# Gabisanth/MaximumAreaCoverageOptimization.jl

Hardware: AMD Instinct MI355X
Metric: MADS objective evals/sec (N UAVs × M fire cells), 1/2/4/8 MI355X (higher is better)
Workload: dtype f64

## Files before the change

### maximumareacoverageoptimization.jl_amd/csrc/k_final.h

```cpp
#pragma once

#include <hip/hip_runtime.h>
#include <stdint.h>

#include "predicate.h"
#include "k_common.h"
#include "k_prep.h"

#pragma clang fp contract(off)

namespace mac {

#ifndef MAC_FIN_C
#define MAC_FIN_C 16
#endif
constexpr int kFinC = MAC_FIN_C;
#ifndef MAC_FIN_MAXBLK
#define MAC_FIN_MAXBLK 256
#endif
constexpr int kFinMaxBlk = MAC_FIN_MAXBLK;
constexpr int kFinThreads = 1024;

struct FinBest {
    double* best;
    uint64_t* mirror;
    uint64_t seq;
    int64_t idx_base;
    unsigned long long* blk;
    unsigned* arrive;
    MadsState* st;
    const double* x;
    double* x_next;
    const int* rp;
    const int* cp;
    uint64_t state;
    int n, ell_max;
    uint64_t done_seq;
    int* hint;
    int* hint_host;
    int nhint;
    int np;
    const unsigned long long* feas;
};

__host__ __device__ __forceinline__ uint64_t mirror_check(uint64_t o, uint64_t i, uint64_t q, uint64_t f = 0)
{
    uint64_t z = o ^ (i * 0x9E3779B97F4A7C15ull) ^ (q * 0xC2B2AE3D27D4EB4Full) ^ (f * 0xD6E8FEB86659FD93ull) ^
                 0x5851F42D4C957F2Dull;
    z = (z ^ (z >> 30)) * 0xBF58476D1CE4E5B9ull;
    z = (z ^ (z >> 27)) * 0x94D049BB133111EBull;
    return z ^ (z >> 31);
}

template <bool kXY = false, bool kMesh = false>
__device__ __forceinline__ void mads_step(const FinBest& fb, double bo, int64_t gidx, int ell, double f)
{
    const int lane = threadIdx.x & (kWave - 1);
    const int n = fb.n;
    const int np = kXY ? fb.np : n;
    const double* __restrict__ x = fb.x;
    double* __restrict__ xn = fb.x_next;
    const bool better = gidx >= 0 && bo < f;
    constexpr int kB = 8;
    const int64_t b = (int64_t)1 << ell;
    const bool plus = gidx < np;
    const int c = better ? fb.cp[plus ? (int)gidx : (int)gidx - np] : 0;
    [[maybe_unused]] const double* gran = nullptr;
    if constexpr (kMesh) gran = fb.st->gran;
    for (int v0 = lane; v0 < n; v0 += kB * kWave) {
        double xv[kB];
        [[maybe_unused]] double gv[kB];
        int rv[kB];
#pragma unroll
        for (int j = 0; j < kB; ++j) {
            const int v = v0 + j * kWave;
            xv[j] = v < n ? x[v] : 0.0;
            rv[j] = better && v < np ? fb.rp[v] : 0;
            if constexpr (kMesh) gv[j] = better && v < np ? gran[v] : 1.0;
        }
#pragma unroll
        for (int j = 0; j < kB; ++j) {
            const int v = v0 + j * kWave;
            if (v >= n) break;
            if (better) {
                double d = ltmads_entry(fb.state, np, b, rv[j], c);
                if constexpr (kMesh) d = gv[j] * d;
                const double moved = plus ? xv[j] + d : xv[j] - d;
                xn[v] = v < np ? moved : xv[j];
            } else {
                xn[v] = xv[j];
            }
        }
    }
    if (lane == 0) {
        const int e = better ? (ell + 1 < fb.ell_max ? ell + 1 : fb.ell_max) : ell - 1;
        fb.st->f = better ? bo : f;
        fb.st->ell = e;
        fb.st->it += 1;
        if (better) fb.st->succ += 1;
    }
}

__device__ __forceinline__ void argmin_take(double& v1, int& i1, double v2, int i2)
{
    if ((i2 >= 0) && (i1 < 0 || v2 < v1 || (v2 == v1 && i2 < i1))) {
        v1 = v2;
        i1 = i2;
    }
}

template <int C = kFinC, bool kXY = false, bool kMesh = false>
__device__ __forceinline__ bool finalize_argmin(const FinBest& fb, double o, int k, bool have)
{
    static_assert(C >= 1 && C <= kWave && (C & (C - 1)) == 0, "C: a power of two up to a wave");
    const int lane = threadIdx.x & (kWave - 1);
    double bv = __builtin_inf();
    int bi = -1;
    if (have && lane < C && o < bv) {
        bv = o;
        bi = k;
    }
#pragma unroll
    for (int off = C / 2; off >= 1; off >>= 1)
        argmin_take(bv, bi, __shfl_xor(bv, off, kWave), __shfl_xor(bi, off, kWave));
    unsigned old = 0;
    if (lane == 0) {
        __hip_atomic_store(fb.blk + 2 * blockIdx.x, __builtin_bit_cast(unsigned long long, bv),
                           __ATOMIC_RELAXED, __HIP_MEMORY_SCOPE_AGENT);
        __hip_atomic_store(fb.blk + 2 * blockIdx.x + 1, (unsigned long long)(long long)bi,
                           __ATOMIC_RELAXED, __HIP_MEMORY_SCOPE_AGENT);
        asm volatile("s_waitcnt vmcnt(0)" ::: "memory");
        old = __hip_atomic_fetch_add(fb.arrive, 1u, __ATOMIC_RELAXED, __HIP_MEMORY_SCOPE_AGENT);
    }
    old = __shfl(old, 0, kWave);
    if (old != gridDim.x - 1) return false;
    const int ell = fb.st ? fb.st->ell : 0;
    const double fcur = fb.st ? fb.st->f : 0.0;
    const int rej = fb.st ? fb.st->skip : 0;
    bv = __builtin_inf();
    bi = -1;
    constexpr int kPer = kFinMaxBlk / kWave;
    unsigned long long v[kPer], ix[kPer];
#pragma unroll
    for (int r = 0; r < kPer; ++r) {
        const unsigned q = lane + r * kWave;
        v[r] = q < gridDim.x ? __hip_atomic_load(fb.blk + 2 * q, __ATOMIC_RELAXED, __HIP_MEMORY_SCOPE_AGENT)
                             : __builtin_bit_cast(unsigned long long, __builtin_inf());
        ix[r] = q < gridDim.x ? __hip_atomic_load(fb.blk + 2 * q + 1, __ATOMIC_RELAXED, __HIP_MEMORY_SCOPE_AGENT)
                              : ~0ull;
    }
    const uint64_t fe = fb.feas ? __hip_atomic_load(fb.feas, __ATOMIC_RELAXED, __HIP_MEMORY_SCOPE_AGENT) : 0ull;
    const bool hl = fb.hint && lane < fb.nhint;
    const int hv = hl ? __hip_atomic_load(fb.hint + lane, __ATOMIC_RELAXED, __HIP_MEMORY_SCOPE_AGENT) : 0;
#pragma unroll
    for (int r = 0; r < kPer; ++r)
        if ((long long)ix[r] >= 0) argmin_take(bv, bi, __builtin_bit_cast(double, v[r]), (int)(long long)ix[r]);
    for (unsigned q = lane + kFinMaxBlk; q < gridDim.x; q += kWave) {
        const unsigned long long vv = __hip_atomic_load(fb.blk + 2 * q, __ATOMIC_RELAXED,
                                                        __HIP_MEMORY_SCOPE_AGENT);
        const unsigned long long xx = __hip_atomic_load(fb.blk + 2 * q + 1, __ATOMIC_RELAXED,
                                                        __HIP_MEMORY_SCOPE_AGENT);
        argmin_take(bv, bi, __builtin_bit_cast(double, vv), (int)(long long)xx);
    }
#pragma unroll
    for (int off = 32; off >= 1; off >>= 1)
        argmin_take(bv, bi, __shfl_xor(bv, off, kWave), __shfl_xor(bi, off, kWave));
    const bool none = bi < 0 || rej;
    const double bo = none ? __builtin_inf() : bv;
    const int64_t gidx = none ? (int64_t)-1 : fb.idx_base + bi;
    if (fb.st && ell < 0) {
        if (lane == 0) __hip_atomic_store(fb.arrive, 0u, __ATOMIC_RELAXED, __HIP_MEMORY_SCOPE_AGENT);
        return true;
    }
    if (fb.st) {
        mads_step<kXY, kMesh>(fb, bo, gidx, ell, fcur);
        if (rej && lane == 0) fb.st->skipped += 1;
    }
    if (lane == 0) {
        unsigned long long* const bw = reinterpret_cast<unsigned long long*>(fb.best);
        __hip_atomic_store(bw, __builtin_bit_cast(unsigned long long, bo), __ATOMIC_RELAXED,
                           __HIP_MEMORY_SCOPE_AGENT);
        __hip_atomic_store(bw + 1, (unsigned long long)gidx, __ATOMIC_RELAXED, __HIP_MEMORY_SCOPE_AGENT);
        __hip_atomic_store(fb.arrive, 0u, __ATOMIC_RELAXED, __HIP_MEMORY_SCOPE_AGENT);
        if (fb.mirror) {
            asm volatile("s_waitcnt vmcnt(0)" ::: "memory");
            const uint64_t o = __builtin_bit_cast(uint64_t, bo);
            const uint64_t ix = (uint64_t)gidx;
            fb.mirror[0] = o;
            fb.mirror[1] = ix;
            fb.mirror[2] = fb.seq;
            if (fb.feas) fb.mirror[4] = fe;
            fb.mirror[3] = mirror_check(o, ix, fb.seq, fe);
            if (fb.st && !(gidx >= 0 && bo < fcur) && ell == 0) fb.mirror[2] = fb.done_seq;
        }
    }
    if (hl) {
        if (fb.hint_host) ((volatile int*)fb.hint_host)[lane] = hv;
        __hip_atomic_store(fb.hint + lane, 0, __ATOMIC_RELAXED, __HIP_MEMORY_SCOPE_AGENT);
    }
    return true;
}

template <bool kXY = false, bool kMesh = false>
__global__ __launch_bounds__(kFinThreads) void finalize_kernel(
    const double* __restrict__ partial, const int* __restrict__ mode, int n_poll, int n_other,
    int K, int N, const int* __restrict__ map, const double* __restrict__ spart,
    const int* __restrict__ ncount, int counts, double w0,
    const double* __restrict__ vp, double* __restrict__ area_out, double* __restrict__ obj_out,
    FinBest fb, uint64_t* ts)
{
    ts_begin(ts);
    double o = __builtin_inf();
    __shared__ double red[kFinThreads / kFinC][kFinC];
    const int t = threadIdx.x, c = t % kFinC, sg = t / kFinC;
    constexpr int SG = kFinThreads / kFinC;
    const int per = (int)(gridDim.x / 8);
    const int cb = per > 0 && gridDim.x % 8 == 0 ? (int)(blockIdx.x % 8) * per + (int)(blockIdx.x / 8)
                                                 : (int)blockIdx.x;
    const int k0 = cb * kFinC;
    const int k = k0 + c;
    const int mv = mode ? *mode : 0;
    const bool cnt_path = counts && spart && map;
    const double vpk = (vp && (sg == 0 || cnt_path) && k < K) ? vp[k] : 0.0;
    if (cnt_path) {
        constexpr int B = 8;
        int pos0[B];
        bool sh0[B];
#pragma unroll
        for (int b = 0; b < B; ++b) {
            const int gb = sg + b * SG;
            const bool in = k < K && gb < n_poll;
            pos0[b] = in ? map[(int64_t)gb * K + k] : -1;
            sh0[b] = in && ncount[gb] > 0;
        }
        const bool skip = vp && !area_out && !(vpk < __builtin_inf());
        if (mv == kModePoll) {
            const unsigned* const crow = reinterpret_cast<const unsigned*>(partial);
            const unsigned* const srow = reinterpret_cast<const unsigned*>(spart);
            __shared__ uint64_t ired[kFinThreads / kFinC][kFinC];
            const int G = n_poll;
            uint64_t a = 0;
            if (k < K && !skip) {
                for (int g = sg; g < G; g += B * SG) {
                    unsigned v[B], sv[B];
                    int pos[B];
                    bool sh[B];
#pragma unroll
                    for (int b = 0; b < B; ++b) {
                        const int gb = g + b * SG;
                        if (g == sg) {
                            pos[b] = pos0[b];
                            sh[b] = sh0[b];
                        } else {
                            pos[b] = gb < G ? map[(int64_t)gb * K + k] : -1;
                            sh[b] = gb < G && ncount[gb] > 0;
                        }
                    }
#pragma unroll
                    for (int b = 0; b < B; ++b) {
                        const int64_t rb = (int64_t)(g + b * SG) * K;
                        v[b] = pos[b] >= 0 ? crow[rb + pos[b]] : 0u;
                        sv[b] = sh[b] ? srow[rb + k] : 0u;
                    }
#pragma unroll
                    for (int b = 0; b < B; ++b) a += (uint64_t)v[b] + sv[b];
                }
            }
            ired[sg][c] = a;
// ... 100 lines not shown
```

### maximumareacoverageoptimization.jl_amd/csrc/k_fiw.h

```cpp
#pragma once

#include <hip/hip_runtime.h>
#include <stdint.h>

#include <type_traits>

#include "predicate.h"
#include "fiw_box.h"
#include "k_common.h"
#include "k_prep.h"
#include "k_index.h"
#include "k_lane.h"
#include "k_poll.h"
#include "k_poll_shared.h"
#include "k_final.h"

#pragma clang fp contract(off)

namespace mac {

constexpr int kFwThreads = 256;
constexpr int kFwWaves = kFwThreads / kWave;
constexpr int kFwPer = 12;
constexpr int kFwMaxK = kFwThreads * kFwPer;
// ... 100 lines not shown
__device__ uint64_t g_diag_f2[8 * 4096];
#define MAC_F2_STAMP(q)                                                                      \
    if (threadIdx.x == 0 && blockIdx.x < 4096) {                                             \
        asm volatile("s_waitcnt vmcnt(0) lgkmcnt(0)" ::: "memory");                          \
        g_diag_f2[8 * blockIdx.x + (q)] = __builtin_amdgcn_s_memrealtime();                  \
    }
#define MAC_F2_NOW() __builtin_amdgcn_s_memrealtime()
#define MAC_F2_PUT(q, v) if (threadIdx.x == 0 && blockIdx.x < 4096) g_diag_f2[8 * blockIdx.x + (q)] = (v)
#else
#define MAC_FW_STAMP(q)
#define MAC_F2_STAMP(q)
#define MAC_F2_NOW() 0
#define MAC_F2_PUT(q, v)
#endif

template <bool C> struct FwAcc { typedef double T; };
template <> struct FwAcc<true> { typedef unsigned T; };

template <bool kCounts, bool kMat, bool kMesh = false>
__global__ __launch_bounds__(kFwThreads) __attribute__((amdgpu_waves_per_eu(2))) void fiw_kernel(
    uint64_t* ts, FwArgs a)
{
    typedef typename FwAcc<kCounts>::T Acc;
    ts_begin(ts);
    CandSrc src = a.src;
    const int N = a.N, K = a.K;
    const Grid g = a.g;
    const int per_xcd = (N + 7) / 8;
    const int i = (int)(blockIdx.x % 8) * per_xcd + (int)(blockIdx.x / 8);
    if (i >= N || !src.resolve_as<kMat>()) {
        ts_end(ts);
        return;
    }
    MAC_FW_STAMP(0);
    __shared__ __attribute__((aligned(16))) uint32_t xbuf[kFwMaxK + 1];
    __shared__ __attribute__((aligned(16))) double tabbuf[kFwMaxK + 1];
    __shared__ __attribute__((aligned(8))) uint16_t zbuf[kFwMaxK + 1];
    constexpr int kSl4 = kFwKPB * 16, kSlx = kFwKPB * 4, kS32 = (kFwCH + 4) * 16, kSix = kFwCH * 4,
                  kSw = kFwCH * 8;
    constexpr int kWB = kSl4 + kSlx + kS32 + kSix + kSw;
    __shared__ __attribute__((aligned(16))) unsigned char wbuf[kWB];
    static_assert(sizeof(uint64_t) * (kFwMaxK + 1) <= kWB, "coverage words fit the walk buffer");
    static_assert(sizeof(int) * (kFwDirect + 1) <= sizeof(double) * (kFwMaxK + 1), "direct table fits");
    constexpr int kFwClr = 4 * kFwThreads;
    __shared__ double2 shp[kFwShE];
    __shared__ double shw[kFwShE];
    __shared__ int shidx[kFwCH];
    __shared__ int rs[kPollRB], rpre[kPollRB + 1];
    __shared__ int nb_id[kFwNbr];
    __shared__ int4 nb_box[kFwNbr];
    __shared__ double nb_b[kFwNbr][3];
    __shared__ double dred[kFwWaves][4];
    __shared__ double sbase[7];
    __shared__ uint8_t scov[kFwKPB];
    __shared__ unsigned ninner;
    __shared__ int ucnt, ncnt, lslot;
    __shared__ int wkeep[kFwR][kFwWaves];
    __shared__ int wshr[kFwR][kFwWaves];
    __shared__ int wsum[kFwWaves];
    uint32_t* const kx = xbuf;
    uint32_t* const poskey = xbuf;
    int* const table = reinterpret_cast<int*>(tabbuf);
    unsigned* const pcnt = reinterpret_cast<unsigned*>(tabbuf);
    double* const pcred = tabbuf;
    uint16_t* const owner_of = reinterpret_cast<uint16_t*>(wbuf);
    uint16_t* const cinfo = zbuf;
    float4* const sl4 = reinterpret_cast<float4*>(wbuf);
    float* const slx = reinterpret_cast<float*>(wbuf + kSl4);
    float4* const s32 = reinterpret_cast<float4*>(wbuf + kSl4 + kSlx);
    int* const six = reinterpret_cast<int*>(wbuf + kSl4 + kSlx + kS32);
    double* const sw = reinterpret_cast<double*>(wbuf + kSl4 + kSlx + kS32 + kSix);
    uint64_t* const Wd = reinterpret_cast<uint64_t*>(wbuf);

    const int tid = threadIdx.x, lane = tid & (kWave - 1), wid = tid / kWave;
    constexpr int P = kFwPer + 1;
    auto kof = [&](int j) { return j < kFwPer ? tid * kFwPer + j : (tid == 0 ? kFwMaxK : K); };

    int4 RG = make_int4(0, -1, 0, -1);
    bool ident;
    int rf0 = 0, rf1 = 0;
    double2 ppr[kFwR];
    double pwr[kFwR];
    int pjg[kFwR];
    {
        const uint32_t* krow = src.keysP + (int64_t)i * src.ldk;
        uint32_t pq[P];
        bool dj[P];
#pragma unroll
        for (int c = 0; c < kFwPer / 4; ++c) {
            const int b0 = tid * kFwPer + 4 * c;
            const uint4 q4 = b0 < src.ldk ? *reinterpret_cast<const uint4*>(krow + b0) : make_uint4(0, 0, 0, 0);
            const uint32_t d4 = a.dead && b0 < src.ldk ? *reinterpret_cast<const uint32_t*>(a.dead + b0) : 0u;
            pq[4 * c] = q4.x;
            pq[4 * c + 1] = q4.y;
            pq[4 * c + 2] = q4.z;
            pq[4 * c + 3] = q4.w;
#pragma unroll
            for (int e = 0; e < 4; ++e) dj[4 * c + e] = ((d4 >> (8 * e)) & 0xFFu) != 0 && b0 + e < K;
        }
        pq[kFwPer] = tid == 0 && K > kFwMaxK ? krow[kFwMaxK] : 0u;
        dj[kFwPer] = tid == 0 && K > kFwMaxK && a.dead && a.dead[kFwMaxK] != 0;
        const double bx = src_val<kMat, kMesh>(src, 0, i, N), by = src_val<kMat, kMesh>(src, 0, N + i, N),
                     br = src_val<kMat, kMesh>(src, 0, 2 * N + i, N);
        double dmx = -__builtin_inf(), dmy = -__builtin_inf(), dmr = -__builtin_inf(), dml = -__builtin_inf();
        for (int q = tid; q < a.npd; q += kFwThreads) {
            const double4 d4 = a.pd[q];
            dmx = fmax(dmx, d4.x);
            dmy = fmax(dmy, d4.y);
            dmr = fmax(dmr, d4.z);
            dml = fmax(dml, d4.w);
        }
        double jb[2][3];
#pragma unroll
        for (int q = 0; q < 2; ++q) {
            const int j = tid + q * kFwThreads;
            const int jc = min(j, N - 1);
            jb[q][0] = j < i ? src_val<kMat, kMesh>(src, 0, jc, N) : 0.0;
            jb[q][1] = j < i ? src_val<kMat, kMesh>(src, 0, N + jc, N) : 0.0;
            jb[q][2] = j < i ? src_val<kMat, kMesh>(src, 0, 2 * N + jc, N) : 0.0;
        }
        if (tid == 0) {
            ucnt = 0;
            ncnt = 0;
            ninner = 0u;
        }
        reinterpret_cast<int4*>(table)[tid] = make_int4(0, 0, 0, 0);
        bool esc = false;
        {
            uint32_t kw[P];
            uint16_t zw[P];
#pragma unroll
            for (int j = 0; j < P; ++j) {
                esc |= kof(j) < K && !dj[j] && pq[j] == kKeyEsc;
                kw[j] = dj[j] ? kDeadWord : pq[j];
                zw[j] = dj[j] ? (uint16_t)0x8000 : (uint16_t)0;
            }
            own_store(kx, kw, tid, K);
            own_store(zbuf, zw, tid, K);
        }
#pragma unroll
        for (int o = 32; o >= 1; o >>= 1) {
            dmx = fmax(dmx, __shfl_xor(dmx, o, kWave));
            dmy = fmax(dmy, __shfl_xor(dmy, o, kWave));
            dmr = fmax(dmr, __shfl_xor(dmr, o, kWave));
            dml = fmax(dml, __shfl_xor(dml, o, kWave));
        }
        if (lane == 0) {
            dred[wid][0] = dmx;
            dred[wid][1] = dmy;
            dred[wid][2] = dmr;
            dred[wid][3] = dml;
        }
        ident = __syncthreads_or(esc);
        MAC_FW_STAMP(1);
#pragma unroll
        for (int q = 0; q < kFwWaves; ++q) {
            dmx = fmax(dmx, dred[q][0]);
            dmy = fmax(dmy, dred[q][1]);
            dmr = fmax(dmr, dred[q][2]);
            dml = fmax(dml, dred[q][3]);
        }
        if (tid == 0) {
            sbase[0] = bx;
            sbase[1] = by;
            sbase[2] = br;
            sbase[3] = dmx;
// ... 14 lines not shown
            auto test = [&](int j, double x0, double y0, double r0) {
                if (box_pre_rejects(bp, x0, y0, r0 + dmr)) return;
                int4 B;
                if (sup_box(x0, y0, r0, dmx, dmy, dmr, g, B) && box_overlap(B, RG)) {
                    const int p = atomicAdd(&ncnt, 1);
                    if (p < kFwNbr) {
                        nb_id[p] = j;
                        nb_box[p] = B;
                        nb_b[p][0] = x0;
                        nb_b[p][1] = y0;
                        nb_b[p][2] = r0;
                    }
                }
            };
#pragma unroll
            for (int q = 0; q < 2; ++q) {
                const int j = tid + q * kFwThreads;
                if (j < i) test(j, jb[q][0], jb[q][1], jb[q][2]);
            }
            for (int j = tid + 2 * kFwThreads; j < i; j += kFwThreads)
                test(j, src_val<kMat, kMesh>(src, 0, j, N), src_val<kMat, kMesh>(src, 0, N + j, N),
                     src_val<kMat, kMesh>(src, 0, 2 * N + j, N));
        }
        MAC_FW_STAMP(12);
        const bool dfits = !ident && dmx >= 0.0 && dmx <= 1023.0 && dmy >= 0.0 && dmy <= 1023.0 &&
                           dmr >= -511.0 && dmr <= 511.0 && dml >= -511.0 && dml <= 511.0;
        const int Dx = dfits ? (int)dmx : 0, Dy = dfits ? (int)dmy : 0;
        const int Dr = dfits ? (int)dmr : 0, Dl = dfits ? (int)dml : 0;
        const int nyd = 2 * Dy + 1, nrd = Dr + Dl + 1;
        const int nslot = dfits && nrd >= 1 ? (2 * Dx + 1) * nyd * nrd : 0;
        bool direct = dfits && nrd >= 1 && (double)Dx == dmx && (double)Dy == dmy && (double)Dr == dmr &&
                      (double)Dl == dml && nslot + 1 <= kFwDirect;
        if (direct && nslot + 1 > kFwClr) {
            for (int q = kFwClr + tid; q <= nslot; q += kFwThreads) table[q] = 0;
            lds_barrier();
        }
        MAC_FW_STAMP(15);
        bool miss = false;
        if (direct) {
            const double tl = __builtin_floor(-br) + 1.0;
            int drlive = !(br == br) ? 512 : tl <= -512.0 ? -512 : tl >= 512.0 ? 512 : (int)tl;
            if (drlive < 512 && !(br + (double)drlive > 0.0)) ++drlive;
            if (drlive > -512 && br + (double)(drlive - 1) > 0.0) --drlive;
            const int sdx = nyd * nrd, sbase0 = (Dx * nyd + Dy) * nrd + Dl;
            const unsigned wx = 2u * (unsigned)Dx, wy = 2u * (unsigned)Dy, wr = (unsigned)(Dr + Dl);
            uint16_t zw[P];
#pragma unroll
            for (int j = 0; j < P; ++j) {
                const int k = kof(j);
                const uint32_t w = pq[j];
                const int dx = (int)(w << 21) >> 21, dy = (int)(w << 10) >> 21, dr = (int)w >> 22;
                const bool live = k < K && !dj[j] && dr >= drlive;
                const bool inr = (unsigned)(dx + Dx) <= wx && (unsigned)(dy + Dy) <= wy &&
                                 (unsigned)(dr + Dl) <= wr;
                miss |= live && !inr;
                const int sl = live && inr ? sbase0 + dx * sdx + dy * nrd + dr : nslot;
                zw[j] = (uint16_t)((dj[j] ? 0x8000 : 0) | sl);
                if (k < K) table[sl] = 1;
            }
            own_store(zbuf, zw, tid, K);
        }
        MAC_FW_STAMP(13);
        {
            const uint64_t mb = __ballot(miss);
            if (lane == 0) wsum[wid] = mb != 0;
            lds_barrier();
            bool any = false;
#pragma unroll
            for (int q = 0; q < kFwWaves; ++q) any |= wsum[q] != 0;
            direct = direct && !any;
            lds_barrier();
        }
        MAC_FW_STAMP(14);
        if (direct) {
            const int per = (nslot + 1 + kFwThreads - 1) / kFwThreads;
            const int s0 = min(tid * per, nslot + 1), s1 = min(s0 + per, nslot + 1);
            int c = 0;
            for (int s = s0; s < s1; ++s) c += table[s];
            const int incl = wave_incl_scan_i32(c, lane);
            if (lane == kWave - 1) wsum[wid] = incl;
            lds_barrier();
            int id = incl - c;
            for (int q = 0; q < wid; ++q) id += wsum[q];
            for (int s = s0; s < s1; ++s) {
                if (table[s]) {
                    uint32_t wk = kDeadWord;
                    if (s < nslot) {
                        const int dr = s % nrd - Dl, t2 = s / nrd;
                        const int dy = t2 % nyd - Dy, dx = t2 / nyd - Dx;
                        wk = key_pack(dx, dy, dr);
                    }
                    poskey[id] = wk;
                    table[s] = id++;
                }
            }
            if (tid == kFwThreads - 1) ucnt = id;
        } else if (!ident) {
            for (int q = tid; q < kFwHash; q += kFwThreads) table[q] = -1;
            lds_barrier();
            constexpr uint32_t mask = kFwHash - 1;
#pragma unroll
            for (int j = 0; j < P; ++j) {
                const int k = kof(j);
                if (k >= K) continue;
                const uint32_t key = kx[k];
                uint32_t s = word_hash(key) & mask;
                for (;;) {
                    int cur = table[s];
                    if (cur < 0) {
                        cur = atomicCAS(&table[s], -1, k);
                        if (cur < 0) break;
                    }
                    if (kx[cur] == key) break;
                    s = (s + 1) & mask;
                }
                zbuf[k] = (uint16_t)((zbuf[k] & 0x8000) | s);
            }
            lds_barrier();
            for (int q = tid; q < kFwHash; q += kFwThreads) {
                const int owner = table[q];
                if (owner >= 0) {
                    const int u = atomicAdd(&ucnt, 1);
                    owner_of[u] = (uint16_t)owner;
                    table[q] = (owner << kFwIdBits) | u;
                }
            }
        }
        lds_barrier();
        MAC_FW_STAMP(2);
        if (rany && tid < kWave) {
            const int nr = min(kPollRB, RG.w - RG.z + 1);
            const int len = tid < nr ? rf1 - rf0 : 0;
            const int incl = wave_incl_scan_i32(len, tid);
            if (tid < nr) {
                rs[tid] = rf0;
                rpre[tid + 1] = incl;
            }
            if (tid == 0) rpre[0] = 0;
        }
        lds_barrier();
        if (rany) {
            const int nr = min(kPollRB, RG.w - RG.z + 1);
            const int nraw = min(kFwCH, rpre[nr]);
#pragma unroll
            for (int r = 0; r < kFwR; ++r) {
                const int qd = tid + r * kFwThreads;
                pjg[r] = -1;
                if (qd < nraw) {
                    int lo = 0, hi = nr - 1;
                    while (lo < hi) {
                        const int mid = (lo + hi + 1) >> 1;
                        if (rpre[mid] <= qd) lo = mid; else hi = mid - 1;
                    }
                    pjg[r] = rs[lo] + (qd - rpre[lo]);
                    ppr[r] = a.xy[pjg[r]];
                    pwr[r] = a.w[pjg[r]];
                }
            }
        }
        const int U0 = ident ? K : ucnt;
        constexpr int PU = (kFwMaxK + 1 + kFwThreads - 1) / kFwThreads;
        uint32_t pkr[PU];
        const bool hashed = !direct && !ident;
#pragma unroll
        for (int q = 0; q < PU; ++q) {
            const int u = tid + q * kFwThreads;
            pkr[q] = hashed && u < U0 ? kx[owner_of[u]] : 0u;
        }
        {
            auto pos_of = [&](uint16_t zb, int k) -> uint16_t {
                const int sl = zb & 0x7FFF;
                const int u = ident ? k : direct ? table[sl] : table[sl] & ((1 << kFwIdBits) - 1);
                return (uint16_t)(u | (zb & 0x8000));
            };
            typedef uint16_t u16x4 __attribute__((ext_vector_type(4)));
            const int b = tid * kFwPer;
            if (b + kFwPer <= K) {
#pragma unroll
                for (int c = 0; c < kFwPer / 4; ++c) {
                    u16x4 q = reinterpret_cast<const u16x4*>(zbuf + b)[c];
                    q.x = pos_of(q.x, b + 4 * c);
                    q.y = pos_of(q.y, b + 4 * c + 1);
                    q.z = pos_of(q.z, b + 4 * c + 2);
                    q.w = pos_of(q.w, b + 4 * c + 3);
                    reinterpret_cast<u16x4*>(cinfo + b)[c] = q;
                }
            } else {
#pragma unroll
                for (int j = 0; j < kFwPer; ++j)
                    if (b + j < K) cinfo[b + j] = pos_of(zbuf[b + j], b + j);
            }
            if (tid == 0 && K > kFwMaxK) cinfo[kFwMaxK] = pos_of(zbuf[kFwMaxK], kFwMaxK);
        }
        lds_barrier();
        if (hashed) {
#pragma unroll
            for (int q = 0; q < PU; ++q)
                if (tid + q * kFwThreads < U0) poskey[tid + q * kFwThreads] = pkr[q];
        }
        for (int u = tid; u < U0; u += kFwThreads) {
            if (kCounts) pcnt[u] = 0u;
            else pcred[u] = 0.0;
        }
        lds_barrier();
    }
    MAC_FW_STAMP(3);
    const int U = ident ? K : ucnt;
    const int nc = ncnt;
    const bool rany = RG.x <= RG.y;
    auto pos_disk = [&](int u) -> DiskRec {
        if (ident) {
            if (cinfo[u] & 0x8000) return inert_disk();
            return make_disk(src_val<kMat, kMesh>(src, u, i, N), src_val<kMat, kMesh>(src, u, N + i, N),
                             src_val<kMat, kMesh>(src, u, 2 * N + i, N));
        }
        return word_disk(poskey[u], sbase[0], sbase[1], sbase[2]);
    };

    auto walk_disk = [&](int u) -> DiskRec {
        DiskRec d;
        if (ident) {
            if (cinfo[u] & 0x8000) return inert_disk();
            d.cx = src_val<kMat, kMesh>(src, u, i, N);
            d.cy = src_val<kMat, kMesh>(src, u, N + i, N);
            d.r = src_val<kMat, kMesh>(src, u, 2 * N + i, N);
        } else {
            const uint32_t w = poskey[u];
            if (w == kDeadWord) return inert_disk();
            float fx, fy, fr;
            key_unpack(w, fx, fy, fr);
            d.cx = sbase[0] + (double)fx;
            d.cy = sbase[1] + (double)fy;
            d.r = sbase[2] + (double)fr;
        }
        d.T = d.r > 0.0 ? d.r * d.r : -1.0;
        return d;
    };
// ... 15 lines not shown
        const double Umax = 0.5 * (double)max(RG.y - RG.x + 1, RG.w - RG.z + 1) * g.S + 2.0 * g.S;
        for (int kb = 0; kb < U; kb += kFwKPB) {
            const int ke = min(U, kb + kFwKPB);
            for (int t = tid; t < kFwKPB; t += kFwThreads) {
                const int u = kb + t;
                PollLane L = inert_lane();
                bool cov = false;
                if (u < ke) {
                    const DiskRec d = walk_disk(u);
                    cov = d.T >= 0.0 && __builtin_isfinite(d.cx) && __builtin_isfinite(d.cy);
                    if (cov) L = poll_lane(d, ox, oy, Umax);
                }
                sl4[t] = make_float4(L.sa, L.sb, L.stm, L.ns);
                slx[t] = L.xp;
                scov[t] = cov ? 1 : 0;
            }
            __syncthreads();
            if (kb == 0) MAC_FW_STAMP(8);
            f32x2 sa[kPollPairs], sb[kPollPairs], st[kPollPairs], ns[kPollPairs];
            float xp[kPollSlots];
            Acc acc[kPollSlots];
            uint32_t live = 0, covm = 0;
#pragma unroll
            for (int u = 0; u < kPollSlots; ++u) {
                const int p = u * kWave + lane;
                const float4 c = sl4[p];
                xp[u] = kb + p < ke ? slx[p] : -1.0f;
                if (kb + p < ke) live |= 1u << u;
                if (kb + p < ke && scov[p]) covm |= 1u << u;
                acc[u] = 0;
                const int j = u >> 1;
                if (u & 1) {
                    sa[j].y = c.x; sb[j].y = c.y; st[j].y = c.z; ns[j].y = c.w;
                } else {
                    sa[j].x = c.x; sb[j].x = c.y; st[j].x = c.z; ns[j].x = c.w;
                }
            }
            const int np = (ke - kb + 2 * kWave - 1) / (2 * kWave);
            for (int rb = RG.z; rb <= RG.w; rb += kPollRB) {
                const int nr = min(kPollRB, RG.w - rb + 1);
                const bool first_rb = kb == 0 && rb == RG.z;
                if (!first_rb) {
                    int rs0 = 0, rs1 = 0;
                    if (rb == RG.z) {
                        if (tid < nr) {
                            rs0 = rf0;
                            rs1 = rf1;
                        }
                    } else if (tid < nr) {
                        const int64_t rowb = (int64_t)(rb + tid) * g.nTx;
                        rs0 = a.off[rowb + RG.x];
                        rs1 = a.off[rowb + RG.y + 1];
                    }
                    __syncthreads();
                    if (tid < kWave) {
                        const int len = tid < nr ? rs1 - rs0 : 0;
                        const int incl = wave_incl_scan_i32(len, tid);
                        if (tid < nr) {
                            rs[tid] = rs0;
                            rpre[tid + 1] = incl;
                        }
                        if (tid == 0) rpre[0] = 0;
                    }
                    __syncthreads();
                }
                const int total = rpre[nr];
                for (int base = 0; base < total; base += kFwCH) {
                    const int nraw = min(kFwCH, total - base);
                    const bool pre = first_rb && base == 0;
                    double2 pr[kFwR];
                    double wr[kFwR];
                    int jg[kFwR];
                    uint64_t bal[kFwR], hbal[kFwR];
#pragma unroll
                    for (int r = 0; r < kFwR; ++r) {
                        const int qd = tid + r * kFwThreads;
                        bool keep = false, inner = false, hs = false;
                        pr[r] = make_double2(0.0, 0.0);
                        wr[r] = 0.0;
                        jg[r] = 0;
                        if (qd < nraw) {
                            const int f = base + qd;
                            int lo = 0, hi = nr - 1;
                            while (lo < hi) {
                                const int mid = (lo + hi + 1) >> 1;
                                if (rpre[mid] <= f) lo = mid; else hi = mid - 1;
                            }
                            if (pre) {
                                jg[r] = pjg[r];
                                pr[r] = ppr[r];
                                wr[r] = pwr[r];
                            } else {
                                jg[r] = rs[lo] + (f - rpre[lo]);
                                pr[r] = a.xy[jg[r]];
                                wr[r] = a.w[jg[r]];
                            }
                            const bool shared = nc > 0 &&
                                entry_shared(nc, nb_box, tile_of(pr[r].x, g.gx0, g.invS, g.nTx), rb + lo);
                            const bool fin = __builtin_isfinite(pr[r].x) && __builtin_isfinite(pr[r].y);
                            keep = !shared && fin;
                            hs = shared && fin;
                            if (keep) {
                                const double ux = pr[r].x - sbase[0], uy = pr[r].y - sbase[1];
                                const double d0 = ux * ux + uy * uy;
                                if (d0 <= rin2) {
                                    keep = false;
                                    inner = true;
                                } else if (d0 >= rout2) {
                                    keep = false;
                                }
                            }
                        }
                        const uint64_t ib = __ballot(inner);
                        if (kb == 0 && lane == 0 && ib) atomicAdd(&ninner, (unsigned)__popcll(ib));
                        bal[r] = __ballot(keep);
                        if (lane == 0) wkeep[r][wid] = __popcll(bal[r]);
                        hbal[r] = __ballot(hs && kb == 0 && hand_ok);
                        if (lane == 0) wshr[r][wid] = __popcll(hbal[r]);
                    }
                    __syncthreads();
                    if (kb == 0 && hand_ok) {
#pragma unroll
                        for (int r = 0; r < kFwR; ++r) {
                            int hd = nsh_walk + __popcll(hbal[r] & ((1ull << lane) - 1));
#pragma unroll
                            for (int w2 = 0; w2 < kFwWaves; ++w2) {
                                if (w2 < wid) hd += wshr[r][w2];
                                nsh_walk += wshr[r][w2];
                            }
                            if (((hbal[r] >> lane) & 1) && hd < kFwShCap) {
                                a.sh.xy[(int64_t)i * kFwShCap + hd] = pr[r];
                                a.sh.w[(int64_t)i * kFwShCap + hd] = wr[r];
                            }
                        }
                    }
                    int n = 0;
#pragma unroll
                    for (int r = 0; r < kFwR; ++r) {
                        int dst = n + __popcll(bal[r] & ((1ull << lane) - 1));
#pragma unroll
                        for (int w2 = 0; w2 < kFwWaves; ++w2) {
                            if (w2 < wid) dst += wkeep[r][w2];
                            n += wkeep[r][w2];
                        }
                        if ((bal[r] >> lane) & 1) {
                            six[dst] = jg[r];
                            sw[dst] = wr[r];
                            const float fu = (float)(pr[r].x - ox), fv = (float)(pr[r].y - oy);
                            s32[dst] = __builtin_isfinite(fu) && __builtin_isfinite(fv)
                                           ? make_float4(__builtin_fmaf(fu, fu, fv * fv), fu, fv, 0.0f)
                                           : make_float4(__builtin_inff(), 0.0f, 0.0f, 0.0f);
                        }
                    }
                    if (tid < ((4 - (n & 3)) & 3)) s32[n + tid] = make_float4(__builtin_inff(), 0.0f, 0.0f, 0.0f);
                    __syncthreads();
                    bool uniform = true;
                    if constexpr (!kCounts) {
                        const uint64_t w0b = __builtin_bit_cast(uint64_t, sw[0]);
                        bool mixed = false;
                        for (int e = tid; e < n; e += kFwThreads) mixed |= __builtin_bit_cast(uint64_t, sw[e]) != w0b;
                        uniform = !__syncthreads_or(mixed);
                    }
                    if (kb == 0 && rb == RG.z && base == 0) MAC_FW_STAMP(9);
                    const int ng = (n + 3) >> 2;
                    float bmin[kPollSlots];
#pragma unroll
                    for (int u = 0; u < kPollSlots; ++u) bmin[u] = __builtin_inff();
                    if (uniform) {
                        f32x2 h[kPollPairs];
// ... 648 lines not shown
```

### maximumareacoverageoptimization.jl_amd/csrc/maxcover.hip

```cpp
#include <hip/hip_runtime.h>
#include <hip/hip_ext.h>
#include <dlfcn.h>
#include <sched.h>
#include <linux/futex.h>
#include <sys/syscall.h>
#include <unistd.h>
#include <hipcub/hipcub.hpp>
#include <immintrin.h>

#include <algorithm>
#include <chrono>
#include <atomic>
#include <cmath>
#include <cstdio>
#include <cstdlib>
#include <cstring>
#include <deque>
#include <mutex>
#include <new>
#include <string>
#include <type_traits>
#include <thread>
#include <vector>

// ... 598 lines not shown
        if (rq.motion)
            hipLaunchKernelGGL(mask_gen_motion_kern(S, rq.cons->sep), dim3((unsigned)K), dim3(kConsBlock),
                               rq.cons->sep ? mask_lds(S) : 0u, r.s, tsm, rq.src, N, *rq.cons, *rq.motion, d_mask);
        else
            hipLaunchKernelGGL(mask_gen_kern(S), dim3((unsigned)K), dim3(kConsBlock), mask_lds(S), r.s, tsm, rq.src,
                               N, *rq.cons, d_mask);
        HCK(hipGetLastError());
    }
    if (rq.prog) {
        uint64_t* tsp = r.ts_role(kRoleProgH, K);
        hipLaunchKernelGGL(prog_h_kernel, dim3((unsigned)K), dim3(kProgBlock), 0, r.s, tsp, rq.src, N, rq.prog->a,
                           rq.prog->h_max, rq.prog->d_h, d_mask, rq.cons ? 1 : 0);
        HCK(hipGetLastError());
    }
    r.d_mask8 = d_mask;
}

static bool fused_history_allows(mac_ctx* ctx, Lane* L)
{
    ensure_hints(L);
    volatile int* hw = (volatile int*)L->h_dc.p;
    int bad_now = -1;
    if (L->last_chain == 2 && hw[8] >= 0) {
        bad_now = hw[8] > kFwCrowdWork || hw[9] > 0 || hw[11] > 0 ? 1 : 0;
        if (ctx->profile) {
            const int64_t id = hw[9];
            ctx->fw_reports.fetch_add(1, std::memory_order_relaxed);
            ctx->fw_ident_sum.fetch_add(id, std::memory_order_relaxed);
            if (id > ctx->fw_ident_max.load(std::memory_order_relaxed))
                ctx->fw_ident_max.store(id, std::memory_order_relaxed);
        }
    }
    else if (L->last_chain == 1 && hw[0] < (1 << 30))
        bad_now = hw[0] > kBitsMinDisks || hw[4] == kModeTiled ? 1 : 0;
    if (bad_now >= 0) {
        uint64_t o = ctx->fused_bad.load(std::memory_order_relaxed);
        while (!ctx->fused_bad.compare_exchange_weak(o, (o << 1) | (uint64_t)bad_now,
                                                     std::memory_order_relaxed)) {
        }
    }
    return ctx->fused_bad.load(std::memory_order_relaxed) == 0;
}

static void key_rows(Lane* L, int N, int K, PrepArgs& pr, CandSrc& src)
{
    const int ldk = keys_ld(K);
    L->keysT.reserve(sizeof(float) * (size_t)4 * N * ldk);
    pr.keysP = L->keysT.as<uint32_t>();
    pr.keysT = L->keysT.as<float>() + (size_t)N * ldk;
    pr.ldk = ldk;
    src.keysP = pr.keysP;
    src.keysT = pr.keysT;
    src.ldk = ldk;
}

static PrepArgs prep_args(const EvalRun& r, int nwg, CandSrc& keyed)
{
    const EvalReq& rq = r.rq;
    PrepArgs pr{};
    pr.src = rq.src;
    pr.N = rq.N;
    pr.K = rq.K;
    pr.pa = PenArgs{rq.d_rmax, rq.d_prev, rq.d_dlimT, rq.d_dlim_raw, rq.tan_half_fov};
    pr.penalty = rq.penalty;
    pr.vp = r.d_vp;
    pr.nchain = nwg;
    pr.skip_failed = rq.d_area ? 0 : 1;
    pr.pair = r.pl.pair ? 1 : 0;
    pr.g = r.ctx->grid;
    pr.feas = rq.d_feas;
    pr.mask8 = r.d_mask8;
    pr.mst_w = rq.fb_mads && r.pl.poll_possible && r.pl.excl && rq.d_prev ? rq.fb_mads->st : nullptr;
    if (r.pl.want_keys) key_rows(r.L, rq.N, rq.K, pr, keyed);
    return pr;
}

static FinBest fin_best(const EvalRun& r, unsigned nfin)
{
    const EvalReq& rq = r.rq;
    Lane* L = r.L;
    FinBest fb{};
    if (!rq.d_best) return fb;
    L->finblk.reserve(2 * sizeof(unsigned long long) * nfin);
    if (L->finarrive.grow(sizeof(unsigned)))
        HCK(hipMemsetAsync(L->finarrive.p, 0, L->finarrive.cap, r.s));
    if (rq.fb_mads) fb = *rq.fb_mads;
    fb.best = rq.d_best;
    fb.mirror = rq.d_mirror;
    fb.seq = rq.mirror_seq;
    fb.idx_base = rq.idx_base;
    fb.blk = L->finblk.as<unsigned long long>();
    fb.arrive = L->finarrive.as<unsigned>();
    fb.feas = rq.d_mirror ? rq.d_feas : nullptr;
    return fb;
}

static void enqueue_fused(EvalRun& r)
{
    const EvalReq& rq = r.rq;
    const EvalPlan& pl = r.pl;
    mac_ctx* ctx = r.ctx;
    Lane* L = r.L;
    hipStream_t s = r.s;
    const int N = rq.N, K = rq.K, counts = pl.counts;
    const bool mat = rq.src.cands != nullptr;
    FwArgs fa{};
    fa.src = rq.src;
    PrepArgs pr = prep_args(r, pl.nprep, fa.src);
    const int ldk = pr.ldk;
    L->pd.reserve(sizeof(double4) * (size_t)pl.nprep);
    L->frows.reserve((counts ? sizeof(unsigned) : sizeof(double)) * (size_t)N * ldk);
    if (L->fwhint.grow(sizeof(int) * kFwHints)) HCK(hipMemsetAsync(L->fwhint.p, 0, L->fwhint.cap, s));
    if (pl.excl) L->dead8.reserve((size_t)ldk + 16);
    L->fwlist.reserve(sizeof(int4) * (size_t)std::max(N, kF2Pre));
    if (L->fwcount.grow(sizeof(int))) HCK(hipMemsetAsync(L->fwcount.p, 0, L->fwcount.cap, s));
    L->fwsxy.reserve(sizeof(double2) * (size_t)N * kFwShCap);
    L->fwsw.reserve(sizeof(double) * (size_t)N * kFwShCap);
    pr.xbase = pl.xbase;
    pr.pd = L->pd.as<double4>();
    pr.dead8 = pl.excl ? L->dead8.as<uint8_t>() : nullptr;
    pr.lreset = L->fwcount.as<int>();
    uint64_t* tsk = r.ts_role(kRolePrep, pl.nprep);
    using hclk = std::chrono::steady_clock;
    hclk::time_point h1, h2, h3;
    if (ctx->host_stats) h1 = hclk::now();
    hipLaunchKernelGGL(prep_kern(pl.prep_fused, pl.mesh), dim3((unsigned)pl.nprep), prep_block(pl.prep_fused), 0, s,
                       tsk, pr);
    HCK(hipGetLastError());
    if (ctx->host_stats) h2 = hclk::now();
    fa.N = N;
    fa.K = K;
    fa.g = ctx->grid;
    fa.dead = pr.dead8;
    fa.pd = pr.pd;
    fa.npd = pl.nprep;
    fa.xy = ctx->xys.as<double2>();
    fa.w = ctx->ws.as<double>();
    fa.off = ctx->off.as<int32_t>();
    fa.counts = counts;
    fa.crow = L->frows.as<unsigned>();
    fa.frow = L->frows.as<double>();
    fa.ldk = ldk;
    fa.hint = L->fwhint.as<int>();
    fa.sh = FwShared{L->fwcount.as<int>(), L->fwlist.as<int4>(), L->fwsxy.as<double2>(), L->fwsw.as<double>()};
    const F2Shared f2s{fa.src, L->fwcount.as<int>(), L->fwlist.as<int4>(), L->fwsxy.as<double2>(),
                       L->fwsw.as<double>(), fa.dead};
    uint64_t* tsw = r.ts_role(kRoleFiw, pl.nfw);
    hipLaunchKernelGGL(fiw_kern(counts, mat, pl.mesh), dim3(pl.nfw), dim3(kFwThreads), 0, s, tsw, fa);
    HCK(hipGetLastError());
    if (ctx->host_stats) h3 = hclk::now();
    FinBest fb = fin_best(r, pl.nfin2);
    if (rq.d_best) {
        fb.hint = L->fwhint.as<int>();
        fb.hint_host = L->d_dc + 8;
        fb.nhint = kFwHints;
    }
    uint64_t* tsf = r.ts_role(kRoleFin2, pl.nfin2);
    hipLaunchKernelGGL(fin2_kern(counts, mat, fb.np != 0, pl.mesh), dim3(pl.nfin2), dim3(kF2Threads), 0, s,
                       counts ? L->frows.as<unsigned>() : nullptr, counts ? nullptr : L->frows.as<double>(),
                       ldk, N, K, ctx->w0, r.d_vp, rq.d_area, rq.d_obj, fb, f2s, tsf);
    HCK(hipGetLastError());
    if (ctx->host_stats) {
        const auto h4 = hclk::now();
        std::lock_guard<std::mutex> lk(ctx->mu);
        ctx->hs_t[0] += std::chrono::duration<double>(h1 - t_poll_entry).count();
        ctx->hs_t[1] += std::chrono::duration<double>(h2 - h1).count();
        ctx->hs_t[2] += std::chrono::duration<double>(h3 - h2).count();
// ... 4021 lines not shown
```

Baseline: 45.98 million.

## Shard finalize arrival counter and cache binary-search results in fiw kernel

The last-block-done counter in the argmin finalize is split into eight cache-line-padded shard counters plus a root counter, to cut same-address atomic contention when many blocks arrive. The fiw kernel also carries each thread's staged binary-search row index in a packed register so the prefetched round skips the repeated search, and computes slot coordinates incrementally instead of with per-slot divisions. In exchange the arrive buffer grows, the reset now touches nine words, and the mirror write ordering moves slightly.

Result: faster. 47.42 million, median of 6 (+3.1%).

```diff
diff --git a/maximumareacoverageoptimization.jl_amd/csrc/k_final.h b/maximumareacoverageoptimization.jl_amd/csrc/k_final.h
--- a/maximumareacoverageoptimization.jl_amd/csrc/k_final.h
+++ b/maximumareacoverageoptimization.jl_amd/csrc/k_final.h
@@ -101,6 +101,16 @@
     }
 }
 
+constexpr int kFinShards = 8;
+constexpr int kFinArriveStride = 128 / (int)sizeof(unsigned);
+constexpr int kFinArriveWords = (kFinShards + 1) * kFinArriveStride;
+
+__device__ __forceinline__ void finalize_arrive_reset(const FinBest& fb, int lane)
+{
+    if (lane <= kFinShards)
+        __hip_atomic_store(fb.arrive + lane * kFinArriveStride, 0u, __ATOMIC_RELAXED, __HIP_MEMORY_SCOPE_AGENT);
+}
+
 __device__ __forceinline__ void argmin_take(double& v1, int& i1, double v2, int i2)
 {
     if ((i2 >= 0) && (i1 < 0 || v2 < v1 || (v2 == v1 && i2 < i1))) {
@@ -123,17 +133,26 @@
 #pragma unroll
     for (int off = C / 2; off >= 1; off >>= 1)
         argmin_take(bv, bi, __shfl_xor(bv, off, kWave), __shfl_xor(bi, off, kWave));
-    unsigned old = 0;
+    unsigned last = 0;
     if (lane == 0) {
         __hip_atomic_store(fb.blk + 2 * blockIdx.x, __builtin_bit_cast(unsigned long long, bv),
                            __ATOMIC_RELAXED, __HIP_MEMORY_SCOPE_AGENT);
         __hip_atomic_store(fb.blk + 2 * blockIdx.x + 1, (unsigned long long)(long long)bi,
                            __ATOMIC_RELAXED, __HIP_MEMORY_SCOPE_AGENT);
         asm volatile("s_waitcnt vmcnt(0)" ::: "memory");
-        old = __hip_atomic_fetch_add(fb.arrive, 1u, __ATOMIC_RELAXED, __HIP_MEMORY_SCOPE_AGENT);
-    }
-    old = __shfl(old, 0, kWave);
-    if (old != gridDim.x - 1) return false;
+        const unsigned grid = gridDim.x, s = blockIdx.x & (kFinShards - 1);
+        const unsigned ns = (grid - s + kFinShards - 1) / kFinShards;
+        const unsigned a = __hip_atomic_fetch_add(fb.arrive + s * kFinArriveStride, 1u, __ATOMIC_RELAXED,
+                                                  __HIP_MEMORY_SCOPE_AGENT);
+        if (a == ns - 1) {
+            const unsigned nroot = grid < (unsigned)kFinShards ? grid : (unsigned)kFinShards;
+            const unsigned r = __hip_atomic_fetch_add(fb.arrive + kFinShards * kFinArriveStride, 1u,
+                                                      __ATOMIC_RELAXED, __HIP_MEMORY_SCOPE_AGENT);
+            last = r == nroot - 1;
+        }
+    }
+    last = __shfl(last, 0, kWave);
+    if (!last) return false;
     const int ell = fb.st ? fb.st->ell : 0;
     const double fcur = fb.st ? fb.st->f : 0.0;
     const int rej = fb.st ? fb.st->skip : 0;
@@ -169,7 +188,7 @@
     const double bo = none ? __builtin_inf() : bv;
     const int64_t gidx = none ? (int64_t)-1 : fb.idx_base + bi;
     if (fb.st && ell < 0) {
-        if (lane == 0) __hip_atomic_store(fb.arrive, 0u, __ATOMIC_RELAXED, __HIP_MEMORY_SCOPE_AGENT);
+        finalize_arrive_reset(fb, lane);
         return true;
     }
     if (fb.st) {
@@ -181,9 +200,11 @@
         __hip_atomic_store(bw, __builtin_bit_cast(unsigned long long, bo), __ATOMIC_RELAXED,
                            __HIP_MEMORY_SCOPE_AGENT);
         __hip_atomic_store(bw + 1, (unsigned long long)gidx, __ATOMIC_RELAXED, __HIP_MEMORY_SCOPE_AGENT);
-        __hip_atomic_store(fb.arrive, 0u, __ATOMIC_RELAXED, __HIP_MEMORY_SCOPE_AGENT);
-        if (fb.mirror) {
-            asm volatile("s_waitcnt vmcnt(0)" ::: "memory");
+    }
+    finalize_arrive_reset(fb, lane);
+    if (fb.mirror) {
+        asm volatile("s_waitcnt vmcnt(0)" ::: "memory");
+        if (lane == 0) {
             const uint64_t o = __builtin_bit_cast(uint64_t, bo);
             const uint64_t ix = (uint64_t)gidx;
             fb.mirror[0] = o;
diff --git a/maximumareacoverageoptimization.jl_amd/csrc/k_fiw.h b/maximumareacoverageoptimization.jl_amd/csrc/k_fiw.h
--- a/maximumareacoverageoptimization.jl_amd/csrc/k_fiw.h
+++ b/maximumareacoverageoptimization.jl_amd/csrc/k_fiw.h
@@ -206,6 +206,8 @@
     double2 ppr[kFwR];
     double pwr[kFwR];
     int pjg[kFwR];
+    [[maybe_unused]] uint32_t plo = 0;
+    static_assert(kPollRB <= 64 && 6 * kFwR <= 32, "plo: 6 bits per staged round");
     {
         const uint32_t* krow = src.keysP + (int64_t)i * src.ldk;
         uint32_t pq[P];
@@ -386,16 +388,20 @@
             lds_barrier();
             int id = incl - c;
             for (int q = 0; q < wid; ++q) id += wsum[q];
+            int dr = s0 % nrd, t2 = s0 / nrd;
+            int dy = t2 % nyd - Dy, dx = t2 / nyd - Dx;
+            dr -= Dl;
             for (int s = s0; s < s1; ++s) {
                 if (table[s]) {
-                    uint32_t wk = kDeadWord;
-                    if (s < nslot) {
-                        const int dr = s % nrd - Dl, t2 = s / nrd;
-                        const int dy = t2 % nyd - Dy, dx = t2 / nyd - Dx;
-                        wk = key_pack(dx, dy, dr);
-                    }
-                    poskey[id] = wk;
+                    poskey[id] = s < nslot ? key_pack(dx, dy, dr) : kDeadWord;
                     table[s] = id++;
+                }
+                if (++dr > Dr) {
+                    dr = -Dl;
+                    if (++dy > Dy) {
+                        dy = -Dy;
+                        ++dx;
+                    }
                 }
             }
             if (tid == kFwThreads - 1) ucnt = id;
@@ -457,6 +463,7 @@
                         if (rpre[mid] <= qd) lo = mid; else hi = mid - 1;
                     }
                     pjg[r] = rs[lo] + (qd - rpre[lo]);
+                    if constexpr (kCounts) plo |= (uint32_t)lo << (6 * r);
                     ppr[r] = a.xy[pjg[r]];
                     pwr[r] = a.w[pjg[r]];
                 }
@@ -638,9 +645,13 @@
                         if (qd < nraw) {
                             const int f = base + qd;
                             int lo = 0, hi = nr - 1;
-                            while (lo < hi) {
-                                const int mid = (lo + hi + 1) >> 1;
-                                if (rpre[mid] <= f) lo = mid; else hi = mid - 1;
+                            if (kCounts && pre) {
+                                lo = (int)((plo >> (6 * r)) & 63u);
+                            } else {
+                                while (lo < hi) {
+                                    const int mid = (lo + hi + 1) >> 1;
+                                    if (rpre[mid] <= f) lo = mid; else hi = mid - 1;
+                                }
                             }
                             if (pre) {
                                 jg[r] = pjg[r];
diff --git a/maximumareacoverageoptimization.jl_amd/csrc/maxcover.hip b/maximumareacoverageoptimization.jl_amd/csrc/maxcover.hip
--- a/maximumareacoverageoptimization.jl_amd/csrc/maxcover.hip
+++ b/maximumareacoverageoptimization.jl_amd/csrc/maxcover.hip
@@ -704,7 +704,7 @@
     FinBest fb{};
     if (!rq.d_best) return fb;
     L->finblk.reserve(2 * sizeof(unsigned long long) * nfin);
-    if (L->finarrive.grow(sizeof(unsigned)))
+    if (L->finarrive.grow(sizeof(unsigned) * kFinArriveWords))
         HCK(hipMemsetAsync(L->finarrive.p, 0, L->finarrive.cap, r.s));
     if (rq.fb_mads) fb = *rq.fb_mads;
     fb.best = rq.d_best;
```
